# Bardli/RMem_ocu

Measured on AMD Instinct MI355X. Metric: frames/sec (whole node) 480p VOS, N=8 memory bank, higher is better.
Workload: dtype bf16; 1 GPU; davis17_480p_r50_N8; clip_frames=80, job_clips=64, clip_feeder=static, objects=3, memory_bank=1+7, gap=5, clips_in_flight_per_gpu=24, clips_per_group=8, step_unit=batch, parallelism=clip-parallel x1, weights=synthetic (no checkpoint offline), hipgraphs=True, frames_from=HBM, encoder_lookahead=2

## Files before the change

include/rmem.h:

```cpp
#ifndef RMEM_H_
#define RMEM_H_

#include <stddef.h>

#ifdef __cplusplus
extern "C" {
#endif

#define RMEM_ABI_VERSION 15

int rmem_abi_version(void);
const char* rmem_last_error_string(void);

typedef struct rmem_conv_desc {
  int H, W, Cin;
  int Ho, Wo, Cout;
  int KH, KW, stride, pad;
  int ldo;
  int ldr;
  int ld2;
  int relu;
  int out_f32;
  int res_f32;
  int ldx;
// ... 122 lines not shown
  const void* att_long; const void* att_short; float* x;
  const void* w_long; const float* b_long; const void* w_short; const float* b_short; void* tgt3;
  const float* ln3_g; const float* ln3_b; const void* w1; const float* b1; void* h1; float* gn_partial;
} rmem_chain_b_desc;
int rmem_lstt_chain_b(const rmem_chain_b_desc* d, void* stream);
int rmem_lstt_chain_b_merged(const rmem_chain_b_desc* d, const rmem_attn_merge* merge, void* stream);

typedef struct rmem_chain_c_desc {
  int L, clips; float eps; int ld_dec;
  float* x;
  const void* h3; const void* w2; const float* b2; const float* dec_g; const float* dec_b; void* dec_out;
  const float* ln1_g; const float* ln1_b; const void* w_qkv; const float* b_qkv; const float* pos_qk; void* qkv;
} rmem_chain_c_desc;
int rmem_lstt_chain_c(const rmem_chain_c_desc* d, void* stream);

int rmem_layernorm(const void* a, int a_is_f32, int lda, const float* gamma, const float* beta, float eps, int M, int C,
                   void* y_bf16, int ldy, float* y_f32, int ldyf, void* stream);

int rmem_patch_merge_ln(const float* x, int H, int W, int C, const float* gamma, const float* beta, float eps,
                        void* y_bf16, void* stream);
int rmem_patch_merge_ln_images(const float* x, int images, int H, int W, int C, const float* gamma, const float* beta, float eps,
                               void* y_bf16, void* stream);

int rmem_window_attn(const void* qkv, const float* qkv_bias, const float* bias_mask_table, void* out, int H, int W,
                     int C, int heads, int shift, void* stream);
int rmem_window_attn_images(const void* qkv, const float* qkv_bias, const float* bias_mask_table, void* out, int images, int H, int W,
                            int C, int heads, int shift, void* stream);

int rmem_add16(const void* a, const void* b, void* y, long long n, void* stream);
int rmem_add16_grouped(int n, const void* const* a, const void* const* b, void* const* y, long long count, void* stream);
// ... 374 lines not shown
int rmem_mem_read_attn_clips_f16(const void* q, int ldq, const void* k_bank, const void* v_bank, long long slot_stride, int ldkv, const rmem_attn_chunk* chunks, int nchunks, int lk_single, const float* pe_cur, const float* pe_mem, int Lq, int heads, void* out, int ldo, float* attn_mass, int T, int nclips, long long q_clip_stride, long long kv_clip_stride, long long out_clip_stride, void* workspace, void* stream);
int rmem_lstt_attn_pair_clips_f16(const void* q, int ldq, const void* k_bank, const void* v_bank, long long slot_stride, int ldkv, const rmem_attn_chunk* chunks, int nchunks, int lk_total, const float* pe_cur, const float* pe_mem, int Lq, int heads, void* out_long, int ldo, float* attn_mass, int T, int nclips, long long q_clip_stride, long long out_clip_stride, const void* k_short, const void* v_short, int lk_short, long long kv_short_clip_stride, void* out_short, long long out_short_clip_stride, void* workspace, void* stream);
int rmem_lstt_attn_pair_clips_deferred_f16(const void* q, int ldq, const void* k_bank, const void* v_bank, long long slot_stride, int ldkv, const rmem_attn_chunk* chunks, int nchunks, int lk_total, const float* pe_cur, const float* pe_mem, int Lq, int heads, void* out_long, int ldo, float* attn_mass, int T, int nclips, long long q_clip_stride, long long out_clip_stride, const void* k_short, const void* v_short, int lk_short, long long kv_short_clip_stride, void* out_short, long long out_short_clip_stride, void* workspace, rmem_attn_merge* merge, void* stream);
int rmem_layernorm256_f16(const void* a, int a_is_f32, int lda, const void* b, int b_is_f32, int ldb, const float* gamma, const float* beta, float eps, int M, void* y_bf16, int ldy, const float* pos, void* ypos_bf16, int ldyp, float* y_f32, int ldyf, void* stream);
int rmem_layernorm_f16(const void* a, int a_is_f32, int lda, const float* gamma, const float* beta, float eps, int M, int C, void* y_bf16, int ldy, float* y_f32, int ldyf, void* stream);
int rmem_patch_merge_ln_f16(const float* x, int H, int W, int C, const float* gamma, const float* beta, float eps, void* y_bf16, void* stream);
int rmem_window_attn_f16(const void* qkv, const float* qkv_bias, const float* bias_mask_table, void* out, int H, int W, int C, int heads, int shift, void* stream);
int rmem_window_attn_images_f16(const void* qkv, const float* qkv_bias, const float* bias_mask_table, void* out, int images, int H, int W, int C, int heads, int shift, void* stream);
int rmem_patch_merge_ln_images_f16(const float* x, int images, int H, int W, int C, const float* gamma, const float* beta, float eps, void* y_bf16, void* stream);
int rmem_add16_f16(const void* a, const void* b, void* y, long long n, void* stream);
int rmem_add16_grouped_f16(int n, const void* const* a, const void* const* b, void* const* y, long long count, void* stream);
int rmem_lstt_chain_a_f16(const rmem_chain_a_desc* d, void* stream);
int rmem_lstt_chain_b_f16(const rmem_chain_b_desc* d, void* stream);
int rmem_lstt_chain_b_merged_f16(const rmem_chain_b_desc* d, const rmem_attn_merge* merge, void* stream);
int rmem_lstt_chain_c_f16(const rmem_chain_c_desc* d, void* stream);
int rmem_layernorm256_pair_f16(const void* a0, const void* b0, void* y0, const void* a1, const void* b1, void* y1, const float* gamma, const float* beta, float eps, int M, void* stream);
int rmem_bneck_block64_f16(const rmem_bneck_block_desc* desc, const void* x, const void* w1, const float* bias1, const void* w2, const float* bias2, const void* w3, const float* bias3, void* y, const void* w1n, const float* bias1n, void* a_next, void* stream);
int rmem_bneck_chain_f16(const rmem_bneck_chain_desc* desc, const void* b, const void* x2, const void* w3, const float* bias3, const void* res, void* y, const void* w1, const float* bias1, void* a2, void* stream);
int rmem_conv1x1_dual_nhwc_f16(const rmem_conv_desc* desc, const void* x, const void* x2, int H2, int W2, int Cin2, int stride2, const void* w_cat, const float* bias, void* y, void* stream);
int rmem_linear_grouped_f16(const rmem_conv_desc* desc, int n, const void* const* x, const void* const* w, const float* const* bias, const void* const* residual, void* const* y, void* stream);
int rmem_groupnorm_nhwc_f16(const void* x, int M, int C, int groups, const float* gamma, const float* beta, float eps, int act, void* y, float* workspace, void* stream);
int rmem_groupnorm_f32_nhwc_f16(const float* x, int M, int C, int groups, const float* gamma, const float* beta, float eps, int act, void* y, float* workspace, void* stream);
int rmem_groupnorm_nhwc_images_f16(const void* x, int images, int M, int C, int groups, const float* gamma, const float* beta, float eps, int act, void* y, float* workspace, void* stream);
int rmem_groupnorm_head_nhwc_images_f16(const void* x, int images, int M, int C, int groups, const float* gamma, const float* beta, float eps, int act, const void* w, const float* bias, int N, float* y, int ldy, float* workspace, void* stream);
int rmem_gn_act_dwconv5x5_nhwc_images_f16(const void* x, int images, int H, int W, int C, int groups, const float* gamma, const float* beta, float eps, int act, const float* w_t, void* y, float* workspace, void* stream);
int rmem_gn_act_dwconv5x5_prestats_nhwc_images_f16(const void* x, int images, int H, int W, int C, int groups, const float* gamma, const float* beta, float eps, int act, const float* w_t, void* y, const float* stats, void* stream);
int rmem_gn_act_dwconv5x5_nhwc_f16(const void* x, int H, int W, int C, int groups, const float* gamma, const float* beta, float eps, int act, const float* w_t, void* y, float* workspace, void* stream);
int rmem_dwconv5x5_nhwc_f16(const void* x, const float* w_t, void* y, int H, int W, int C, void* stream);
int rmem_image_ptrs_to_nhwc4p_f16(const float* const* img_ptrs, void* out_padded, int images, int H, int W, void* stream);
int rmem_conv3x3_direct_f16(const void* x, int images, int H, int W, int C, const void* w, const float* bias, int relu, void* y, void* stream);
// ... 24 lines not shown
```

rmem_ocu_amd/_lib.py:

```python
from __future__ import annotations

import ctypes as C
import os
import subprocess

_HERE = os.path.dirname(os.path.abspath(__file__))
LIB_PATH = os.environ.get('RMEM_LIB_PATH') or os.path.join(_HERE, 'librmem_hip.so')
ABI_VERSION = 15


class RmemError(RuntimeError):
    pass


class ConvDesc(C.Structure):
    _fields_ = [(n, C.c_int) for n in ('H', 'W', 'Cin', 'Ho', 'Wo', 'Cout', 'KH', 'KW', 'stride', 'pad',
                                       'ldo', 'ldr', 'ld2', 'relu', 'out_f32', 'res_f32', 'ldx', 'batch', 'act_begin',
                                       'res_up_h', 'res_up_w', 'res_up_align')]


class GemmPlan(C.Structure):
    _fields_ = [(n, C.c_int) for n in ('family', 'tile', 'ring', 'is1x1', 'fast', 'splits', 'steps_per_split', 'xcd_ny',
                                       'grid_x', 'grid_y', 'grid_z', 'threads')]

# ... 83 lines not shown
    _fields_ = [('ngroups', _i), ('heads', _i), ('Lq', _i), ('reserved', _i), ('opart', _vp), ('mlg', _vp), ('opart_cs', _ll), ('mlg_cs', _ll)]


def _desc(name, ints, ptrs):
    return type(name, (C.Structure,), {'_fields_': [(ints[0], _i), (ints[1], _i), ('eps', _f), (ints[2], _i)] + [(n, _vp) for n in ptrs]})


ChainA = _desc('ChainA', ('L', 'clips', 'reserved'),
               ('att', 'x', 'w_proj', 'b_proj', 'ln2_g', 'ln2_b', 'curr_v', 'w_q', 'b_q', 'curr_q', 'short_k', 'short_v', 'ln4_g', 'ln4_b',
                'k4', 'v4'))
ChainB = _desc('ChainB', ('L', 'clips', 'gn_splits'),
               ('att_long', 'att_short', 'x', 'w_long', 'b_long', 'w_short', 'b_short', 'tgt3', 'ln3_g', 'ln3_b', 'w1', 'b1', 'h1',
                'gn_partial'))
ChainC = _desc('ChainC', ('L', 'clips', 'ld_dec'),
               ('x', 'h3', 'w2', 'b2', 'dec_g', 'dec_b', 'dec_out', 'ln1_g', 'ln1_b', 'w_qkv', 'b_qkv', 'pos_qk', 'qkv'))
SIGNATURES = {
    'rmem_abi_version': (_i, []),
    'rmem_last_error_string': (C.c_char_p, []),
    'rmem_conv_workspace_bytes': (C.c_size_t, [C.POINTER(ConvDesc)]),
    'rmem_conv2d_nhwc': (_i, [C.POINTER(ConvDesc), _vp, _vp, _vp, _vp, _vp, _vp, _vp, _vp]),
    'rmem_conv_plan': (_i, [C.POINTER(ConvDesc), _i, _i, _i, C.POINTER(GemmPlan)]),
    'rmem_attn_workspace_bytes': (C.c_size_t, [_i, _i, _i]),
    'rmem_mem_read_attn': (_i, [_vp, _i, _vp, _vp, _ll, _i, _vp, _i, _i, _vp, _vp, _i, _i, _vp, _i, _vp, _i, _vp, _vp]),
    'rmem_profile_start': (_i, [_i]),
    'rmem_profile_stop': (_i, [C.POINTER(C.c_double), C.POINTER(C.c_double), C.POINTER(_i)]),
    'rmem_layernorm256': (_i, [_vp, _i, _i, _vp, _i, _i, _vp, _vp, _f, _i, _vp, _i, _vp, _vp, _i, _vp, _i, _vp]),
    'rmem_layernorm': (_i, [_vp, _i, _i, _vp, _vp, _f, _i, _i, _vp, _i, _vp, _i, _vp]),
    'rmem_patch_merge_ln': (_i, [_vp, _i, _i, _i, _vp, _vp, _f, _vp, _vp]),
    'rmem_window_attn': (_i, [_vp, _vp, _vp, _vp, _i, _i, _i, _i, _i, _vp]),
    'rmem_window_attn_images': (_i, [_vp, _vp, _vp, _vp, _i, _i, _i, _i, _i, _i, _vp]),
    'rmem_patch_merge_ln_images': (_i, [_vp, _i, _i, _i, _i, _vp, _vp, _f, _vp, _vp]),
    'rmem_add16': (_i, [_vp, _vp, _vp, _ll, _vp]),
    'rmem_add16_grouped': (_i, [_i, C.POINTER(_vp), C.POINTER(_vp), C.POINTER(_vp), _ll, _vp]),
    'rmem_layernorm256_pair': (_i, [_vp, _vp, _vp, _vp, _vp, _vp, _vp, _vp, _f, _i, _vp]),
    'rmem_lstt_chain_waves': (_i, []),
    'rmem_lstt_chain_rows': (_i, [_i, _i, _i]),
    'rmem_lstt_chain_a': (_i, [C.POINTER(ChainA), _vp]),
    'rmem_lstt_chain_b': (_i, [C.POINTER(ChainB), _vp]),
    'rmem_lstt_chain_b_merged': (_i, [C.POINTER(ChainB), C.POINTER(AttnMerge), _vp]),
    'rmem_lstt_chain_c': (_i, [C.POINTER(ChainC), _vp]),
    'rmem_conv1x1_dual_nhwc': (_i, [C.POINTER(ConvDesc), _vp, _vp, _i, _i, _i, _i, _vp, _vp, _vp, _vp]),
    'rmem_bneck_chain': (_i, [C.POINTER(BneckChainDesc), _vp, _vp, _vp, _vp, _vp, _vp, _vp, _vp, _vp, _vp]),
    'rmem_bneck_block64': (_i, [C.POINTER(BneckBlockDesc), _vp, _vp, _vp, _vp, _vp, _vp, _vp, _vp, _vp, _vp, _vp, _vp]),
    'rmem_linear_grouped': (_i, [C.POINTER(ConvDesc), _i, C.POINTER(_vp), C.POINTER(_vp), C.POINTER(_vp), C.POINTER(_vp), C.POINTER(_vp), _vp]),
    'rmem_groupnorm_workspace_bytes': (C.c_size_t, [_i]),
    'rmem_groupnorm_nhwc': (_i, [_vp, _i, _i, _i, _vp, _vp, _f, _i, _vp, _vp, _vp]),
    'rmem_groupnorm_f32_nhwc': (_i, [_vp, _i, _i, _i, _vp, _vp, _f, _i, _vp, _vp, _vp]),
    'rmem_groupnorm_nhwc_images': (_i, [_vp, _i, _i, _i, _i, _vp, _vp, _f, _i, _vp, _vp, _vp]),
    'rmem_groupnorm_head_nhwc_images': (_i, [_vp, _i, _i, _i, _i, _vp, _vp, _f, _i, _vp, _vp, _i, _vp, _i, _vp, _vp]),
    'rmem_gn_act_dwconv5x5_nhwc_images': (_i, [_vp, _i, _i, _i, _i, _i, _vp, _vp, _f, _i, _vp, _vp, _vp, _vp]),
    'rmem_gn_act_dwconv5x5_prestats_nhwc_images': (_i, [_vp, _i, _i, _i, _i, _i, _vp, _vp, _f, _i, _vp, _vp, _vp, _vp]),
    'rmem_bilinear_nhwc_images': (_i, [_vp, _vp, _i, _i, _i, _i, _i, _i, _i, _vp]),
    'rmem_mem_read_attn_clips': (_i, [_vp, _i, _vp, _vp, _ll, _i, _vp, _i, _i, _vp, _vp, _i, _i, _vp, _i, _vp, _i, _i, _ll, _ll, _ll, _vp, _vp]),
    'rmem_lstt_attn_pair_clips': (_i, [_vp, _i, _vp, _vp, _ll, _i, _vp, _i, _i, _vp, _vp, _i, _i, _vp, _i, _vp, _i, _i, _ll, _ll,
                                       _vp, _vp, _i, _ll, _vp, _ll, _vp, _vp]),
# ... 107 lines not shown
    'rmem_jpeg_entropy_decode': (_i, [_vp, _vp, _i, _i, C.POINTER(JpegPlan), _vp, _vp, _vp, _vp]),
    'rmem_jpeg_coef_to_rgb': (_i, [_vp, _i, _i, C.POINTER(JpegPlan), _vp, _vp, _vp]),
    'rmem_jpeg_decode_batch': (_i, [_vp, _vp, _i, _i, C.POINTER(JpegPlan), _vp, _vp, _vp, _vp, _vp]),
    'rmem_jpeg_encode_header': (_i, [_i, _i, _i, _i, _vp, _i, C.POINTER(_i), _vp]),
    'rmem_jpeg_encode_bound': (C.c_size_t, [_i, _i]),
    'rmem_jpeg_encode_workspace_bytes': (C.c_size_t, [_i, _i, _i]),
    'rmem_jpeg_encode_rgb8': (_i, [_vp, _vp, _vp, _i, _i, _i, _i, _vp, _vp, _vp, _vp, _vp]),
    'rmem_overlay_rgb8': (_i, [_vp, _vp, _vp, _i, _i, _i, _i, _vp, _vp]),
    'rmem_graph_begin': (_i, [_vp]),
    'rmem_graph_end': (_i, [_vp, C.POINTER(_vp)]),
    'rmem_graph_launch': (_i, [_vp, _vp]),
    'rmem_graph_destroy': (_i, [_vp]),
}

F16_TWINS = ('rmem_conv2d_nhwc', 'rmem_mem_read_attn', 'rmem_mem_read_attn_clips', 'rmem_lstt_attn_pair_clips', 'rmem_lstt_attn_pair_clips_deferred', 'rmem_layernorm256', 'rmem_layernorm', 'rmem_patch_merge_ln',
             'rmem_window_attn', 'rmem_window_attn_images', 'rmem_patch_merge_ln_images', 'rmem_add16', 'rmem_add16_grouped', 'rmem_layernorm256_pair', 'rmem_lstt_chain_a', 'rmem_lstt_chain_b', 'rmem_lstt_chain_b_merged', 'rmem_lstt_chain_c', 'rmem_conv1x1_dual_nhwc', 'rmem_bneck_chain', 'rmem_bneck_block64', 'rmem_label_id_embed', 'rmem_image_ptrs_to_nhwc4p', 'rmem_stem7x7s2', 'rmem_stem7x7s2_pool', 'rmem_conv3x3_c64_direct', 'rmem_conv3x3_direct', 'rmem_linear_grouped',
             'rmem_groupnorm_nhwc', 'rmem_groupnorm_f32_nhwc', 'rmem_groupnorm_nhwc_images', 'rmem_groupnorm_head_nhwc_images',
             'rmem_gn_act_dwconv5x5_nhwc_images', 'rmem_gn_act_dwconv5x5_prestats_nhwc_images', 'rmem_gn_act_dwconv5x5_nhwc', 'rmem_dwconv5x5_nhwc', 'rmem_image_to_nhwc8',
             'rmem_image_to_nhwc8_images', 'rmem_image_ptrs_to_nhwc8', 'rmem_ingest_rgb8', 'rmem_maxpool3x3s2_nhwc', 'rmem_maxpool3x3s2_nhwc_images', 'rmem_bilinear_nhwc',
             'rmem_bilinear_nhwc_images', 'rmem_label_to_onehot16', 'rmem_label_to_onehot16_images', 'rmem_gated_attn', 'rmem_local_gated_attn', 'rmem_gated_attn_clips', 'rmem_local_gated_attn_clips')
SIGNATURES.update({n + '_f16': SIGNATURES[n] for n in F16_TWINS})

_lib = None


def build(force: bool = False) -> str:
    src = os.path.join(_HERE, 'csrc')
    if force:
        subprocess.run(['make', '-C', src, 'clean'], check=True, capture_output=True)
    r = subprocess.run(['make', '-C', src, '-j8'], capture_output=True, text=True)
    if r.returncode != 0:
# ... 26 lines not shown
```

rmem_ocu_amd/csrc/rowchain.hip:

```cpp
#include "common.h"
#include "lds_dma.h"
#include "../../include/rmem.h"
#include <stdlib.h>

namespace {

#ifndef RMEM_CHAIN_WAVES
#define RMEM_CHAIN_WAVES 8
#endif
constexpr int NW = RMEM_CHAIN_WAVES;
constexpr int NT = 64 * NW;
constexpr int JT = 16 / NW;
constexpr int WC = 256 / NW;
constexpr int RW = 32 / NW;
constexpr int XS = 260;
constexpr int PF = 16 / JT;

__device__ __forceinline__ f32x4 ld4(const float* p) { return *reinterpret_cast<const f32x4*>(p); }
__device__ __forceinline__ e16x4 cvt4(f32x4 v) { return e16x4{(e16)v[0], (e16)v[1], (e16)v[2], (e16)v[3]}; }
__device__ __forceinline__ f32x4 up4(e16x4 v) { return f32x4{(float)v[0], (float)v[1], (float)v[2], (float)v[3]}; }

typedef __attribute__((ext_vector_type(2))) unsigned u32x2;
typedef __attribute__((ext_vector_type(4))) unsigned u32x4;
#if defined(__HIP_DEVICE_COMPILE__)
__device__ __forceinline__ void st8(rsrc_t r, int off, e16x4 v) { __builtin_amdgcn_raw_buffer_store_b64(__builtin_bit_cast(u32x2, v), r, off, 0, 0); }
__device__ __forceinline__ void st16(rsrc_t r, int off, f32x4 v) { __builtin_amdgcn_raw_buffer_store_b128(__builtin_bit_cast(u32x4, v), r, off, 0, 0); }
#else
__device__ inline void st8(rsrc_t, int, e16x4) {}
__device__ inline void st16(rsrc_t, int, f32x4) {}
#endif

template <int BM, int NP>
__device__ __forceinline__ void stage_tile(e16* A16, int p0, const e16* src, long ld, int nrows) {
  constexpr int NI = NP * BM * 8 / NT;
  static_assert(NP * BM * 8 % NT == 0, "the chunks must divide among the threads");
  const int ch = threadIdx.x & 7;
  e16x8 v[NI];
#pragma unroll
  for (int k = 0; k < NI; ++k) {
    const int i = (threadIdx.x + k * NT) >> 3, row = i % BM;
    v[k] = *reinterpret_cast<const e16x8*>(src + min(row, nrows - 1) * ld + ch * 8 + (i / BM) * 64);
  }
#pragma unroll
  for (int k = 0; k < NI; ++k) {
    const int i = (threadIdx.x + k * NT) >> 3, row = i % BM;
    *reinterpret_cast<e16x8*>(&A16[(p0 + i / BM) * (BM * 64) + swz(row, ch)]) = v[k];
  }
}

template <int BM>
__device__ __forceinline__ void put_a(e16* A16, int p0, int row, int lane, e16x4 v) {
  *reinterpret_cast<e16x4*>(&A16[(p0 + (lane >> 4)) * (BM * 64) + swz(row, (lane & 15) >> 1) + (lane & 1) * 4]) = v;
}

constexpr float MERGE_NEG_BIG = -1.0e30f;
template <int BM>
__device__ __forceinline__ void stage_merged(e16* A16, const rmem_attn_merge& mg, int nrows, int L) {
#pragma clang fp contract(off)
  constexpr int TQ = NT / BM;
  constexpr int HP = TQ >= 8 ? 1 : 8 / TQ;
  constexpr int GP = TQ > 8 ? 64 / TQ : 8;
  const int ql = threadIdx.x % BM, hh = threadIdx.x / BM;
// ... 432 lines not shown
    dump_acc(X, acc, wave, lane);
    if (nb < 2) { wq = wstream((const e16*)d.w_qkv, nb + 1, wave, 8); b_preload(ring, wq, lane); }
    __syncthreads();
#pragma unroll
    for (int h = 0; h < NH; ++h)
#pragma unroll
      for (int rr = 0; rr < RW; ++rr) {
        f32x4 v = ld4(&X[wrow(h, wave, rr) * XS + c0]);
        v += bq[nb];
        v += pos[h].r[rr];
        st8(rqkv, row_off(blk, h, wave, rr, 768, nb * 256 + c0, 2), cvt4(v));
      }
  }
}

#ifndef RMEM_F16
}
extern "C" int rmem_lstt_chain_waves(void) { return NW; }
extern "C" int rmem_lstt_chain_rows(int L, int clips, int cus) { return (long)((L + 31) / 32) * clips > cus ? 64 : 32; }
namespace {
#endif
bool al16(const void* p) { return p == nullptr || ((uintptr_t)p % 16) == 0; }

int chain_rows(int L, int clips) {
  if (const char* e = getenv("RMEM_CHAIN_ROWS")) {
    const int x = atoi(e);
    return x == 32 || x == 64 ? x : 0;
  }
  static int cus = 0;
  if (cus <= 0) {
    int dev = 0, n = 0;
    if (hipGetDevice(&dev) != hipSuccess || hipDeviceGetAttribute(&n, hipDeviceAttributeMultiprocessorCount, dev) != hipSuccess || n <= 0)
      return 32;
    cus = n;
  }
  return rmem_lstt_chain_rows(L, clips, cus);
}

}

extern "C" int RMEM_API(rmem_lstt_chain_a)(const rmem_chain_a_desc* d, void* stream) {
  RMEM_REQUIRE(d && d->L > 0 && d->clips >= 1 && (long)d->L * d->clips < (1L << 20), "rmem_lstt_chain_a: bad geometry (rows must stay below 2^20)");
  RMEM_REQUIRE(d->att && d->x && d->w_proj && d->b_proj && d->ln2_g && d->ln2_b && d->curr_v && d->w_q && d->b_q && d->curr_q && d->short_k &&
               d->short_v && d->ln4_g && d->ln4_b && d->k4 && d->v4, "rmem_lstt_chain_a: null argument");
  RMEM_REQUIRE(al16(d->att) && al16(d->x) && al16(d->w_proj) && al16(d->w_q) && al16(d->curr_v) && al16(d->curr_q) && al16(d->short_k) &&
               al16(d->short_v) && al16(d->k4) && al16(d->v4) && al16(d->b_proj) && al16(d->b_q) && al16(d->ln2_g) && al16(d->ln2_b) &&
               al16(d->ln4_g) && al16(d->ln4_b), "rmem_lstt_chain_a: operands must be 16-byte aligned");
  const int bm = chain_rows(d->L, d->clips);
  RMEM_REQUIRE(bm, "rmem_lstt_chain_a: RMEM_CHAIN_ROWS must be 32 or 64");
  const dim3 grid((d->L + bm - 1) / bm, d->clips);
  if (bm == 64) hipLaunchKernelGGL(k_chain_a<64>, grid, dim3(NT), 0, (hipStream_t)stream, *d);
// ... 53 lines not shown
  const int bm = chain_rows(d->L, d->clips);
  RMEM_REQUIRE(bm, "rmem_lstt_chain_c: RMEM_CHAIN_ROWS must be 32 or 64");
  const dim3 grid((d->L + bm - 1) / bm, d->clips);
  hipStream_t s = (hipStream_t)stream;
  if (bm == 64) {
    if (ffn2 && next) hipLaunchKernelGGL((k_chain_c<64, true, true>), grid, dim3(NT), 0, s, *d);
    else if (ffn2) hipLaunchKernelGGL((k_chain_c<64, true, false>), grid, dim3(NT), 0, s, *d);
    else hipLaunchKernelGGL((k_chain_c<64, false, true>), grid, dim3(NT), 0, s, *d);
  } else {
    if (ffn2 && next) hipLaunchKernelGGL((k_chain_c<32, true, true>), grid, dim3(NT), 0, s, *d);
    else if (ffn2) hipLaunchKernelGGL((k_chain_c<32, true, false>), grid, dim3(NT), 0, s, *d);
    else hipLaunchKernelGGL((k_chain_c<32, false, true>), grid, dim3(NT), 0, s, *d);
  }
  return rmem_check_launch("rmem_lstt_chain_c");
}
```

rmem_ocu_amd/group_runtime.py:

```python
from __future__ import annotations

from typing import Dict, List, Optional, Tuple

import os

import torch

from . import ops
from .encoder_batch import BatchEncoder, SwinBatchEncoder
from .pack import R50_BLOCKS, R50_STRIDES
from .runtime import BF16, D_MODEL, F32, FFN, HEADS, MAX_CHUNKS, PLAIN_CHUNKS, _out, sine_pos_emb, temporal_slots


class GroupRuntime:
    deaot = False
    max_rows = MAX_CHUNKS
    bank_kw = bank_vw = D_MODEL
    dec_cin = 4 * D_MODEL

    def __init__(self, P: Dict[str, torch.Tensor], in_hw: Tuple[int, int], bank_slots: int, device, clips: int,
                 num_lstt: int = 3, align_corners: bool = True, num_classes: int = 11, lookahead: int = 4):
        if ('g0.qvu.w' in P) != self.deaot:
            raise ops.RmemError('GroupRuntime covers the AOTL paths (ResNet-50 / Swin-B), group_runtime_deaot.GroupRuntimeDeAOT the R50-DeAOTL path')
        self.swin = 'pe.w' in P
        self.chain = not os.environ.get('RMEM_NO_CHAIN')
        self.pair_attn = not os.environ.get('RMEM_NO_PAIR_ATTN')
        self.merge_fold = not os.environ.get('RMEM_NO_MERGE_FOLD')
        self.P, self.dev, self.NL, self.B = P, device, num_lstt, clips
        self.dt = P['proj.w'].dtype
        self.align, self.nc = align_corners, num_classes
        H, W = in_hw
        self.H, self.W = H, W
        B = clips
        if self.swin:
            if H % 4 or W % 4:
                raise ops.RmemError('Swin-B path: network size must be a multiple of 4 (the evaluator makes it a multiple of 16)')
            self.H4, self.W4 = H // 4, W // 4
            self.H8, self.W8 = (self.H4 + 1) // 2, (self.W4 + 1) // 2
            self.H16, self.W16 = (self.H8 + 1) // 2, (self.W8 + 1) // 2
            self.enc_ch = (128, 256, 512)
        else:
            self.H2, self.W2 = _out(H, 7, 2, 3), _out(W, 7, 2, 3)
# ... 326 lines not shown
            o = [ops.label_id_embed(labels, P['idbank.w'], P['idbank.b'], self.lab_net, self.id_emb, Hs=hs, Ws=ws, H=self.H, W=self.W, K=k,
                                    stride=s, pad=p, ncls=self.nc, images=B)]
        else:
            o = [ops.label_to_onehot16(labels, self.onehot, Hs=hs, Ws=ws, Hd=self.H, Wd=self.W, ncls=self.nc, images=B)]
            o.append(self._conv(self.onehot, P['idbank.w'], P['idbank.b'], self.id_emb, H=self.H, W=self.W, Cin=16, Cout=D_MODEL,
                                KH=k, KW=k, stride=s, pad=p))
        self._prog[key] = o
        return o

    def prog_update(self, append: bool) -> list:
        key = f'update_{int(append)}'
        if key in self._prog:
            return self._prog[key]
        P, NL, L, C, B = self.P, self.NL, self.L, D_MODEL, self.B
        R = B * L
        o = [ops.add16_grouped(self.tgt3 + (self.curr_V if append else []), [self.id_emb] * (NL * (2 if append else 1)),
                                  self.tmpA + (self.tmpB if append else []), R * C)]
        w = lambda nm: [P[f'l{i}.{nm}.w'] for i in range(NL)]
        b = lambda nm: [P[f'l{i}.{nm}.b'] for i in range(NL)]
        o.append(ops.linear_grouped(self.tgt3, w('linear_QMem'), b('linear_QMem'), self.short_K, M=R, K=C, N=C))
        o.append(ops.linear_grouped(self.tmpA, w('linear_VMem'), b('linear_VMem'), self.short_V, M=R, K=C, N=C))
        if append:
            o.append(ops.linear_grouped(self.tmpB, w('linear_V'), b('linear_V'), self.new_V, M=R, K=C, N=C))
            for i in range(NL):
                o.append(self._scatter(self.curr_Q[i], self.bank_K[i]))
                o.append(self._scatter(self.new_V[i], self.bank_V[i]))
        self._prog[key] = o
        return o


# ... 6 lines not shown
```

rmem_ocu_amd/ops.py:

```python
from __future__ import annotations

import ctypes as C
import os
from typing import Dict, Optional, Sequence

import torch

from . import _lib
from ._lib import AttnChunk, ConvDesc, RmemError

BF16 = torch.bfloat16
F16 = torch.float16
F32 = torch.float32
E16 = (BF16, F16)


def _fn(name: str, dt):
    if dt not in E16:
        raise RmemError(f'{name}: 16-bit operands must be bfloat16 or float16, got {dt}')
    return getattr(_lib.lib(), name + ('_f16' if dt == F16 else ''))


def _first16(*ts):
    for t in ts:
# ... 199 lines not shown
                  dict(att_long=att_long, att_short=att_short, x=x, w_long=w_long, b_long=b_long, w_short=w_short, b_short=b_short, tgt3=tgt3,
                       ln3_g=ln3[0], ln3_b=ln3[1], w1=w1, b1=b1, h1=h1, gn_partial=gn_partial), dt, () if merge is None else (merge,))


def lstt_chain_c(*, L, clips, x, dt, h3=None, w2=None, b2=None, dec_norm=(None, None), dec_out=None, ld_dec=0, ln1=(None, None), w_qkv=None,
                 b_qkv=None, pos_qk=None, qkv=None, eps=1e-5) -> Op:
    R = clips * L
    assert x.dtype == F32 and x.numel() >= R * 256
    assert h3 is None or (h3.dtype == dt and h3.numel() >= R * 1024 and w2.numel() == 262144 and dec_out.numel() >= (R - 1) * ld_dec + 256)
    assert w_qkv is None or (w_qkv.numel() == 196608 and pos_qk.dtype == F32 and pos_qk.numel() >= R * 768 and qkv.dtype == dt and qkv.numel() >= R * 768)
    return _chain('rmem_lstt_chain_c', _lib.ChainC, (L, clips, eps, ld_dec),
                  dict(x=x, h3=h3, w2=w2, b2=b2, dec_g=dec_norm[0], dec_b=dec_norm[1], dec_out=dec_out, ln1_g=ln1[0], ln1_b=ln1[1], w_qkv=w_qkv,
                       b_qkv=b_qkv, pos_qk=pos_qk, qkv=qkv), dt)


def attn_workspace(Lq: int, heads: int, nchunks: int, device, nclips: int = 1) -> torch.Tensor:
    n = nclips * _lib.lib().rmem_attn_workspace_bytes(Lq, heads, nchunks)
    return torch.empty(n // 4, dtype=F32, device=device)


def make_chunk_table(chunks: Sequence[Sequence[int]]) -> torch.Tensor:
    t = torch.zeros(len(chunks), 8, dtype=torch.int32)
    for i, c in enumerate(chunks):
        t[i, :5] = torch.tensor(list(c), dtype=torch.int32)
    return t


def mem_read_attn(q, k_bank, v_bank, out, workspace, *, Lq, heads=8, ldq, ldkv, ldo, slot_stride=0, chunks=None,
                  nchunks=1, lk_single=0, pe_cur=None, pe_mem=None, mass=None, T=0, nclips=1, q_cs=0, kv_cs=0, out_cs=0) -> Op:
    _dev(q, k_bank, v_bank, out, workspace, chunks, pe_cur, pe_mem, mass)
# ... 493 lines not shown
```

rmem_ocu_amd/pack.py:

```python
from __future__ import annotations

from typing import Dict

import torch

import threading

BN_EPS = 1e-5
_DT = torch.bfloat16
_PACK_LOCK = threading.Lock()
R50_BLOCKS = (3, 4, 6)
R50_STRIDES = (1, 2, 2)


def _conv_w(w: torch.Tensor, cin_pad: int = 0) -> torch.Tensor:
    cout, cin, kh, kw = w.shape
    w = w.permute(0, 2, 3, 1)
    if cin_pad and cin_pad > cin:
        w = torch.nn.functional.pad(w, (0, cin_pad - cin))
    return w.contiguous().to(_DT)


def pack_frag(w: torch.Tensor, waves: int = 0) -> torch.Tensor:
    if not waves:
# ... 136 lines not shown
        norm(d + '.ln1', s + '.norm1')
        put(d + '.self_qk.w', torch.cat([sd[s + '.self_attn.linear_Q.weight'], sd[s + '.self_attn.linear_K.weight']], 0).float().to(_DT))
        put(d + '.self_qk.b', torch.cat([sd[s + '.self_attn.linear_Q.bias'], sd[s + '.self_attn.linear_K.bias']], 0).float())
        put(d + '.self_qkv.w', torch.cat([sd[s + '.self_attn.linear_Q.weight'], sd[s + '.self_attn.linear_K.weight'],
                                          sd[s + '.self_attn.linear_V.weight']], 0).float().to(_DT))
        put(d + '.self_qkv.b', torch.cat([sd[s + '.self_attn.linear_Q.bias'], sd[s + '.self_attn.linear_K.bias'],
                                          sd[s + '.self_attn.linear_V.bias']], 0).float())
        lin(d + '.self_proj', s + '.self_attn.projection')
        norm(d + '.ln2', s + '.norm2')
        for nm in ('linear_Q', 'linear_V', 'linear_QMem', 'linear_VMem', 'linear1', 'linear2'):
            lin(f'{d}.{nm}', f'{s}.{nm}')
        norm(d + '.ln4', s + '.norm4')
        lin(d + '.long_proj', s + '.long_term_attn.projection')
        lin(d + '.short_proj', s + '.short_term_attn.projection')
        norm(d + '.ln3', s + '.norm3')
        for nm in ('self_proj', 'linear_Q', 'long_proj', 'short_proj', 'linear1', 'linear2', 'self_qkv'):
            put(f'{d}.{nm}.wf', pack_frag(P[f'{d}.{nm}.w']))
        norm(d + '.gn', s + '.activation.gn')
        put(d + '.dw.w', sd[s + '.activation.conv.weight'].float().view(-1, 25).t())
        norm(f'dec_norm{i}', f'LSTT.decoder_norms.{i}')

    for nm in ('conv_in', 'conv_16x', 'conv_8x', 'conv_4x'):
        put(f'dec.{nm}.w', _conv_w(sd[f'decoder.{nm}.conv.weight'].float())); put(f'dec.{nm}.b', sd[f'decoder.{nm}.conv.bias'].float())
        norm(f'dec.{nm}.gn', f'decoder.{nm}.gn')
    for nm in ('adapter_16x', 'adapter_8x', 'adapter_4x', 'conv_out'):
        put(f'dec.{nm}.w', _conv_w(sd[f'decoder.{nm}.weight'].float())); put(f'dec.{nm}.b', sd[f'decoder.{nm}.bias'].float())

    put('idbank.w', _conv_w(sd['patch_wise_id_bank.weight'].float(), cin_pad=16)); put('idbank.b', sd['patch_wise_id_bank.bias'].float())
    put('pe_cur', sd['cur_pos_emb'].float().view(-1)); put('pe_mem', sd['mem_pos_emb'].float())
    return P
```

Before: 3480 frames/s.

## Fuse LSTT memory-update linears, id add and bank append into one chain kernel

```diff
diff --git a/include/rmem.h b/include/rmem.h
--- a/include/rmem.h
+++ b/include/rmem.h
@@ -160,6 +160,15 @@
 } rmem_chain_c_desc;
 int rmem_lstt_chain_c(const rmem_chain_c_desc* d, void* stream);
 
+typedef struct rmem_chain_u_desc {
+  int L, clips, layers, append;
+  long long slot_stride; const int* append_slots; const void* id_emb;
+  const void* tgt3[4]; const void* curr_v[4]; const void* curr_q[4];
+  void* short_k[4]; void* short_v[4]; void* new_v[4]; void* bank_k[4]; void* bank_v[4];
+  const void* w_qmem[4]; const float* b_qmem[4]; const void* w_vmem[4]; const float* b_vmem[4]; const void* w_v[4]; const float* b_v[4];
+} rmem_chain_u_desc;
+int rmem_lstt_chain_update(const rmem_chain_u_desc* d, void* stream);
+
 int rmem_layernorm(const void* a, int a_is_f32, int lda, const float* gamma, const float* beta, float eps, int M, int C,
                    void* y_bf16, int ldy, float* y_f32, int ldyf, void* stream);
 
@@ -564,6 +573,7 @@
 int rmem_lstt_chain_b_f16(const rmem_chain_b_desc* d, void* stream);
 int rmem_lstt_chain_b_merged_f16(const rmem_chain_b_desc* d, const rmem_attn_merge* merge, void* stream);
 int rmem_lstt_chain_c_f16(const rmem_chain_c_desc* d, void* stream);
+int rmem_lstt_chain_update_f16(const rmem_chain_u_desc* d, void* stream);
 int rmem_layernorm256_pair_f16(const void* a0, const void* b0, void* y0, const void* a1, const void* b1, void* y1, const float* gamma, const float* beta, float eps, int M, void* stream);
 int rmem_bneck_block64_f16(const rmem_bneck_block_desc* desc, const void* x, const void* w1, const float* bias1, const void* w2, const float* bias2, const void* w3, const float* bias3, void* y, const void* w1n, const float* bias1n, void* a_next, void* stream);
 int rmem_bneck_chain_f16(const rmem_bneck_chain_desc* desc, const void* b, const void* x2, const void* w3, const float* bias3, const void* res, void* y, const void* w1, const float* bias1, void* a2, void* stream);
diff --git a/rmem_ocu_amd/_lib.py b/rmem_ocu_amd/_lib.py
--- a/rmem_ocu_amd/_lib.py
+++ b/rmem_ocu_amd/_lib.py
@@ -121,6 +121,15 @@
                 'gn_partial'))
 ChainC = _desc('ChainC', ('L', 'clips', 'ld_dec'),
                ('x', 'h3', 'w2', 'b2', 'dec_g', 'dec_b', 'dec_out', 'ln1_g', 'ln1_b', 'w_qkv', 'b_qkv', 'pos_qk', 'qkv'))
+
+
+class ChainU(C.Structure):
+    PER_LAYER = ('tgt3', 'curr_v', 'curr_q', 'short_k', 'short_v', 'new_v', 'bank_k', 'bank_v', 'w_qmem', 'b_qmem', 'w_vmem', 'b_vmem',
+                 'w_v', 'b_v')
+    _fields_ = [('L', _i), ('clips', _i), ('layers', _i), ('append', _i), ('slot_stride', _ll), ('append_slots', _vp), ('id_emb', _vp)] + \
+               [(n, _vp * 4) for n in PER_LAYER]
+
+
 SIGNATURES = {
     'rmem_abi_version': (_i, []),
     'rmem_last_error_string': (C.c_char_p, []),
@@ -146,6 +155,7 @@
     'rmem_lstt_chain_b': (_i, [C.POINTER(ChainB), _vp]),
     'rmem_lstt_chain_b_merged': (_i, [C.POINTER(ChainB), C.POINTER(AttnMerge), _vp]),
     'rmem_lstt_chain_c': (_i, [C.POINTER(ChainC), _vp]),
+    'rmem_lstt_chain_update': (_i, [C.POINTER(ChainU), _vp]),
     'rmem_conv1x1_dual_nhwc': (_i, [C.POINTER(ConvDesc), _vp, _vp, _i, _i, _i, _i, _vp, _vp, _vp, _vp]),
     'rmem_bneck_chain': (_i, [C.POINTER(BneckChainDesc), _vp, _vp, _vp, _vp, _vp, _vp, _vp, _vp, _vp, _vp]),
     'rmem_bneck_block64': (_i, [C.POINTER(BneckBlockDesc), _vp, _vp, _vp, _vp, _vp, _vp, _vp, _vp, _vp, _vp, _vp, _vp]),
@@ -283,7 +293,7 @@
 }
 
 F16_TWINS = ('rmem_conv2d_nhwc', 'rmem_mem_read_attn', 'rmem_mem_read_attn_clips', 'rmem_lstt_attn_pair_clips', 'rmem_lstt_attn_pair_clips_deferred', 'rmem_layernorm256', 'rmem_layernorm', 'rmem_patch_merge_ln',
-             'rmem_window_attn', 'rmem_window_attn_images', 'rmem_patch_merge_ln_images', 'rmem_add16', 'rmem_add16_grouped', 'rmem_layernorm256_pair', 'rmem_lstt_chain_a', 'rmem_lstt_chain_b', 'rmem_lstt_chain_b_merged', 'rmem_lstt_chain_c', 'rmem_conv1x1_dual_nhwc', 'rmem_bneck_chain', 'rmem_bneck_block64', 'rmem_label_id_embed', 'rmem_image_ptrs_to_nhwc4p', 'rmem_stem7x7s2', 'rmem_stem7x7s2_pool', 'rmem_conv3x3_c64_direct', 'rmem_conv3x3_direct', 'rmem_linear_grouped',
+             'rmem_window_attn', 'rmem_window_attn_images', 'rmem_patch_merge_ln_images', 'rmem_add16', 'rmem_add16_grouped', 'rmem_layernorm256_pair', 'rmem_lstt_chain_a', 'rmem_lstt_chain_b', 'rmem_lstt_chain_b_merged', 'rmem_lstt_chain_c', 'rmem_lstt_chain_update', 'rmem_conv1x1_dual_nhwc', 'rmem_bneck_chain', 'rmem_bneck_block64', 'rmem_label_id_embed', 'rmem_image_ptrs_to_nhwc4p', 'rmem_stem7x7s2', 'rmem_stem7x7s2_pool', 'rmem_conv3x3_c64_direct', 'rmem_conv3x3_direct', 'rmem_linear_grouped',
              'rmem_groupnorm_nhwc', 'rmem_groupnorm_f32_nhwc', 'rmem_groupnorm_nhwc_images', 'rmem_groupnorm_head_nhwc_images',
              'rmem_gn_act_dwconv5x5_nhwc_images', 'rmem_gn_act_dwconv5x5_prestats_nhwc_images', 'rmem_gn_act_dwconv5x5_nhwc', 'rmem_dwconv5x5_nhwc', 'rmem_image_to_nhwc8',
              'rmem_image_to_nhwc8_images', 'rmem_image_ptrs_to_nhwc8', 'rmem_ingest_rgb8', 'rmem_maxpool3x3s2_nhwc', 'rmem_maxpool3x3s2_nhwc_images', 'rmem_bilinear_nhwc',
diff --git a/rmem_ocu_amd/csrc/rowchain.hip b/rmem_ocu_amd/csrc/rowchain.hip
--- a/rmem_ocu_amd/csrc/rowchain.hip
+++ b/rmem_ocu_amd/csrc/rowchain.hip
@@ -31,21 +31,34 @@
 #endif
 
 template <int BM, int NP>
+struct Tile {
+  static_assert(NP * BM * 8 % NT == 0, "the chunks must divide among the threads");
+  static constexpr int NI = NP * BM * 8 / NT;
+  e16x8 v[NI];
+};
+template <int BM, int NP>
+__device__ __forceinline__ Tile<BM, NP> load_tile(const e16* src, long ld, int nrows) {
+  const int ch = threadIdx.x & 7;
+  Tile<BM, NP> t;
+#pragma unroll
+  for (int k = 0; k < Tile<BM, NP>::NI; ++k) {
+    const int i = (threadIdx.x + k * NT) >> 3, row = i % BM;
+    t.v[k] = *reinterpret_cast<const e16x8*>(src + min(row, nrows - 1) * ld + ch * 8 + (i / BM) * 64);
+  }
+  return t;
+}
+template <int BM, int NP>
+__device__ __forceinline__ void put_tile(e16* A16, int p0, const Tile<BM, NP>& t) {
+  const int ch = threadIdx.x & 7;
+#pragma unroll
+  for (int k = 0; k < Tile<BM, NP>::NI; ++k) {
+    const int i = (threadIdx.x + k * NT) >> 3, row = i % BM;
+    *reinterpret_cast<e16x8*>(&A16[(p0 + i / BM) * (BM * 64) + swz(row, ch)]) = t.v[k];
+  }
+}
+template <int BM, int NP>
 __device__ __forceinline__ void stage_tile(e16* A16, int p0, const e16* src, long ld, int nrows) {
-  constexpr int NI = NP * BM * 8 / NT;
-  static_assert(NP * BM * 8 % NT == 0, "the chunks must divide among the threads");
-  const int ch = threadIdx.x & 7;
-  e16x8 v[NI];
-#pragma unroll
-  for (int k = 0; k < NI; ++k) {
-    const int i = (threadIdx.x + k * NT) >> 3, row = i % BM;
-    v[k] = *reinterpret_cast<const e16x8*>(src + min(row, nrows - 1) * ld + ch * 8 + (i / BM) * 64);
-  }
-#pragma unroll
-  for (int k = 0; k < NI; ++k) {
-    const int i = (threadIdx.x + k * NT) >> 3, row = i % BM;
-    *reinterpret_cast<e16x8*>(&A16[(p0 + i / BM) * (BM * 64) + swz(row, ch)]) = v[k];
-  }
+  put_tile<BM, NP>(A16, p0, load_tile<BM, NP>(src, ld, nrows));
 }
 
 template <int BM>
@@ -508,6 +521,127 @@
   }
 }
 
+constexpr int OS = 260;
+
+template <int NI>
+__device__ __forceinline__ void add_id(e16x8 (&o)[NI], const e16x8 (&a)[NI], const e16x8 (&b)[NI]) {
+#pragma unroll
+  for (int k = 0; k < NI; ++k)
+#pragma unroll
+    for (int j = 0; j < 8; ++j) o[k][j] = (e16)((float)a[k][j] + (float)b[k][j]);
+}
+
+template <int MT>
+__device__ __forceinline__ void put_out(e16* O, const f32x4 (&acc)[MT][JT], const float (&bias)[JT], int wave, int lane) {
+  const int fr = lane & 15, fc = lane >> 4;
+#pragma unroll
+  for (int i = 0; i < MT; ++i)
+#pragma unroll
+    for (int j = 0; j < JT; ++j)
+#pragma unroll
+      for (int q = 0; q < 4; ++q) O[(i * 16 + fc * 4 + q) * OS + wave * WC + j * 16 + fr] = (e16)(acc[i][j][q] + bias[j]);
+}
+
+template <int BM>
+__device__ __forceinline__ void store_out(const e16* O, rsrc_t r, const Blk& blk, int wave, int lane) {
+#pragma unroll
+  for (int h = 0; h < BM / 32; ++h)
+#pragma unroll
+    for (int rr = 0; rr < RW; ++rr)
+      st8(r, row_off(blk, h, wave, rr, 256, lane * 4, 2), *reinterpret_cast<const e16x4*>(&O[wrow(h, wave, rr) * OS + lane * 4]));
+}
+
+__device__ __forceinline__ void load_bias(float (&b)[JT], const float* bias, int wave, int lane) {
+#pragma unroll
+  for (int j = 0; j < JT; ++j) b[j] = bias[wave * WC + j * 16 + (lane & 15)];
+}
+
+template <int BM, bool APPEND>
+__global__ __launch_bounds__(NT) void k_chain_u(rmem_chain_u_desc d) {
+  constexpr int MT = BM / 16, PANEL = BM * 64;
+  typedef Tile<BM, 4> T4;
+  __shared__ __attribute__((aligned(16))) char smem[4 * PANEL * 2 + BM * OS * 2];
+  e16* A16 = reinterpret_cast<e16*>(smem);
+  e16* O = reinterpret_cast<e16*>(smem + 4 * PANEL * 2);
+  const int lane = threadIdx.x & 63, wave = __builtin_amdgcn_readfirstlane(threadIdx.x >> 6);
+  const Blk blk = my_rows<BM>(d.L);
+  const Blk inclip = {blk.nrows, (long)blockIdx.x * BM};
+  const long rows = (long)d.clips * d.L;
+  const int l0 = gridDim.z > 1 ? blockIdx.z : 0, l1 = gridDim.z > 1 ? l0 + 1 : d.layers;
+  const int slot = APPEND ? d.append_slots[blockIdx.y] : -1;
+  const long slot_off = slot >= 0 ? slot * d.slot_stride : 0, slot_bytes = slot >= 0 ? (long)d.L * 512 : 0;
+  const T4 id = load_tile<BM, 4>((const e16*)d.id_emb + blk.g0 * 256, 256, blk.nrows);
+  T4 t = load_tile<BM, 4>((const e16*)d.tgt3[l0] + blk.g0 * 256, 256, blk.nrows);
+  BRing ring;
+  f32x4 acc[MT][JT];
+  const e16* w = wstream((const e16*)d.w_qmem[l0], 0, wave, 8);
+  b_preload(ring, w, lane);
+  for (int l = l0; l < l1; ++l) {
+    const rsrc_t rsk = make_rsrc(d.short_k[l], rows * 512), rsv = make_rsrc(d.short_v[l], rows * 512);
+    float bqm[JT], bvm[JT], bv[JT];
+    load_bias(bqm, d.b_qmem[l], wave, lane);
+    load_bias(bvm, d.b_vmem[l], wave, lane);
+    T4 cv, cq;
+    if (APPEND) {
+      load_bias(bv, d.b_v[l], wave, lane);
+      cv = load_tile<BM, 4>((const e16*)d.curr_v[l] + blk.g0 * 256, 256, blk.nrows);
+      cq = load_tile<BM, 4>((const e16*)d.curr_q[l] + blk.g0 * 256, 256, blk.nrows);
+    }
+    put_tile<BM, 4>(A16, 0, t);
+    __syncthreads();
+    zero_acc(acc);
+    gemm_rows<BM, 4>(A16, 0, w, ring, acc, lane);
+    w = wstream((const e16*)d.w_vmem[l], 0, wave, 8);
+    b_preload(ring, w, lane);
+    __syncthreads();
+    {
+      T4 s;
+      add_id(s.v, t.v, id.v);
+      put_tile<BM, 4>(A16, 0, s);
+    }
+    put_out(O, acc, bqm, wave, lane);
+    if (l + 1 < l1) t = load_tile<BM, 4>((const e16*)d.tgt3[l + 1] + blk.g0 * 256, 256, blk.nrows);
+    __syncthreads();
+    store_out<BM>(O, rsk, blk, wave, lane);
+    zero_acc(acc);
+    gemm_rows<BM, 4>(A16, 0, w, ring, acc, lane);
+    if (APPEND || l + 1 < l1) {
+      w = wstream((const e16*)(APPEND ? d.w_v[l] : d.w_qmem[l + 1]), 0, wave, 8);
+      b_preload(ring, w, lane);
+    }
+    __syncthreads();
+    put_out(O, acc, bvm, wave, lane);
+    if (APPEND) {
+      T4 s;
+      add_id(s.v, cv.v, id.v);
+      put_tile<BM, 4>(A16, 0, s);
+    }
+    __syncthreads();
+    store_out<BM>(O, rsv, blk, wave, lane);
+    if (APPEND) {
+      const rsrc_t rnv = make_rsrc(d.new_v[l], rows * 512);
+      const rsrc_t rbk = make_rsrc((const e16*)d.bank_k[l] + slot_off, slot_bytes), rbv = make_rsrc((const e16*)d.bank_v[l] + slot_off, slot_bytes);
+#pragma unroll
+      for (int k = 0; k < T4::NI; ++k) {
+        const int i = (threadIdx.x + k * NT) >> 3, row = i % BM;
+        const int off = row < blk.nrows ? (int)(((inclip.g0 + row) * 256 + (i / BM) * 64 + (threadIdx.x & 7) * 8) * 2) : OOB;
+        st16(rbk, off, __builtin_bit_cast(f32x4, cq.v[k]));
+      }
+      zero_acc(acc);
+      gemm_rows<BM, 4>(A16, 0, w, ring, acc, lane);
+      if (l + 1 < l1) {
+        w = wstream((const e16*)d.w_qmem[l + 1], 0, wave, 8);
+        b_preload(ring, w, lane);
+      }
+      __syncthreads();
+      put_out(O, acc, bv, wave, lane);
+      __syncthreads();
+      store_out<BM>(O, rnv, blk, wave, lane);
+      store_out<BM>(O, rbv, inclip, wave, lane);
+    }
+  }
+}
+
 #ifndef RMEM_F16
 }
 extern "C" int rmem_lstt_chain_waves(void) { return NW; }
@@ -516,19 +650,24 @@
 #endif
 bool al16(const void* p) { return p == nullptr || ((uintptr_t)p % 16) == 0; }
 
+int device_cus() {
+  static int cus = 0;
+  if (cus <= 0) {
+    int dev = 0, n = 0;
+    if (hipGetDevice(&dev) != hipSuccess || hipDeviceGetAttribute(&n, hipDeviceAttributeMultiprocessorCount, dev) != hipSuccess || n <= 0)
+      return 0;
+    cus = n;
+  }
+  return cus;
+}
+
 int chain_rows(int L, int clips) {
   if (const char* e = getenv("RMEM_CHAIN_ROWS")) {
     const int x = atoi(e);
     return x == 32 || x == 64 ? x : 0;
   }
-  static int cus = 0;
-  if (cus <= 0) {
-    int dev = 0, n = 0;
-    if (hipGetDevice(&dev) != hipSuccess || hipDeviceGetAttribute(&n, hipDeviceAttributeMultiprocessorCount, dev) != hipSuccess || n <= 0)
-      return 32;
-    cus = n;
-  }
-  return rmem_lstt_chain_rows(L, clips, cus);
+  const int cus = device_cus();
+  return cus ? rmem_lstt_chain_rows(L, clips, cus) : 32;
 }
 
 }
@@ -612,3 +751,36 @@
   }
   return rmem_check_launch("rmem_lstt_chain_c");
 }
+
+extern "C" int RMEM_API(rmem_lstt_chain_update)(const rmem_chain_u_desc* d, void* stream) {
+  RMEM_REQUIRE(d && d->L > 0 && d->clips >= 1 && (long)d->L * d->clips < (1L << 20), "rmem_lstt_chain_update: bad geometry (rows must stay below 2^20)");
+  RMEM_REQUIRE(d->layers >= 1 && d->layers <= 4, "rmem_lstt_chain_update: 1 to 4 layers");
+  RMEM_REQUIRE(d->id_emb && al16(d->id_emb), "rmem_lstt_chain_update: id_emb must be given and 16-byte aligned");
+  const bool append = d->append != 0;
+  RMEM_REQUIRE(!append || (d->append_slots && d->slot_stride >= (long long)d->L * 256 && d->slot_stride % 8 == 0),
+               "rmem_lstt_chain_update: an append needs append_slots and slot_stride >= L * 256 elements (a multiple of 8)");
+  for (int i = 0; i < d->layers; ++i) {
+    RMEM_REQUIRE(d->tgt3[i] && d->short_k[i] && d->short_v[i] && d->w_qmem[i] && d->b_qmem[i] && d->w_vmem[i] && d->b_vmem[i],
+                 "rmem_lstt_chain_update: null argument");
+    RMEM_REQUIRE(al16(d->tgt3[i]) && al16(d->short_k[i]) && al16(d->short_v[i]) && al16(d->w_qmem[i]) && al16(d->w_vmem[i]),
+                 "rmem_lstt_chain_update: operands must be 16-byte aligned");
+    if (!append) continue;
+    RMEM_REQUIRE(d->curr_v[i] && d->curr_q[i] && d->new_v[i] && d->bank_k[i] && d->bank_v[i] && d->w_v[i] && d->b_v[i],
+                 "rmem_lstt_chain_update: null argument of an append");
+    RMEM_REQUIRE(al16(d->curr_v[i]) && al16(d->curr_q[i]) && al16(d->new_v[i]) && al16(d->bank_k[i]) && al16(d->bank_v[i]) && al16(d->w_v[i]),
+                 "rmem_lstt_chain_update: operands must be 16-byte aligned");
+  }
+  const int bm = chain_rows(d->L, d->clips);
+  RMEM_REQUIRE(bm, "rmem_lstt_chain_update: RMEM_CHAIN_ROWS must be 32 or 64");
+  const int nx = (d->L + bm - 1) / bm;
+  const dim3 grid(nx, d->clips, (long)nx * d->clips * d->layers <= device_cus() ? d->layers : 1);
+  hipStream_t s = (hipStream_t)stream;
+  if (bm == 64) {
+    if (append) hipLaunchKernelGGL((k_chain_u<64, true>), grid, dim3(NT), 0, s, *d);
+    else hipLaunchKernelGGL((k_chain_u<64, false>), grid, dim3(NT), 0, s, *d);
+  } else {
+    if (append) hipLaunchKernelGGL((k_chain_u<32, true>), grid, dim3(NT), 0, s, *d);
+    else hipLaunchKernelGGL((k_chain_u<32, false>), grid, dim3(NT), 0, s, *d);
+  }
+  return rmem_check_launch("rmem_lstt_chain_update");
+}
diff --git a/rmem_ocu_amd/group_runtime.py b/rmem_ocu_amd/group_runtime.py
--- a/rmem_ocu_amd/group_runtime.py
+++ b/rmem_ocu_amd/group_runtime.py
@@ -26,6 +26,7 @@
         self.chain = not os.environ.get('RMEM_NO_CHAIN')
         self.pair_attn = not os.environ.get('RMEM_NO_PAIR_ATTN')
         self.merge_fold = not os.environ.get('RMEM_NO_MERGE_FOLD')
+        self.update_chain = os.environ.get('RMEM_NO_UPDATE_CHAIN') != '1'
         self.P, self.dev, self.NL, self.B = P, device, num_lstt, clips
         self.dt = P['proj.w'].dtype
         self.align, self.nc = align_corners, num_classes
@@ -382,6 +383,14 @@
             return self._prog[key]
         P, NL, L, C, B = self.P, self.NL, self.L, D_MODEL, self.B
         R = B * L
+        if self.chain and self.update_chain:
+            p = lambda nm, k: [P[f'l{i}.{nm}.{k}'] for i in range(NL)]
+            kw = dict(curr_v=self.curr_V, curr_q=self.curr_Q, new_v=self.new_V, bank_k=self.bank_K, bank_v=self.bank_V,
+                      w_v=p('linear_V', 'wf'), b_v=p('linear_V', 'b'), append_slots=self.append_slots, slot_stride=L * C) if append else {}
+            self._prog[key] = [ops.lstt_chain_update(L=L, clips=B, id_emb=self.id_emb, tgt3=self.tgt3, short_k=self.short_K, short_v=self.short_V,
+                                                     w_qmem=p('linear_QMem', 'wf'), b_qmem=p('linear_QMem', 'b'),
+                                                     w_vmem=p('linear_VMem', 'wf'), b_vmem=p('linear_VMem', 'b'), **kw)]
+            return self._prog[key]
         o = [ops.add16_grouped(self.tgt3 + (self.curr_V if append else []), [self.id_emb] * (NL * (2 if append else 1)),
                                   self.tmpA + (self.tmpB if append else []), R * C)]
         w = lambda nm: [P[f'l{i}.{nm}.w'] for i in range(NL)]
diff --git a/rmem_ocu_amd/ops.py b/rmem_ocu_amd/ops.py
--- a/rmem_ocu_amd/ops.py
+++ b/rmem_ocu_amd/ops.py
@@ -237,6 +237,34 @@
                        b_qkv=b_qkv, pos_qk=pos_qk, qkv=qkv), dt)
 
 
+def lstt_chain_update(*, L, clips, id_emb, tgt3, short_k, short_v, w_qmem, b_qmem, w_vmem, b_vmem, curr_v=None, curr_q=None, new_v=None,
+                      bank_k=None, bank_v=None, w_v=None, b_v=None, append_slots=None, slot_stride=0) -> Op:
+    dt = id_emb.dtype
+    R, n = clips * L, len(tgt3)
+    append = curr_v is not None
+    per_layer = dict(tgt3=tgt3, curr_v=curr_v, curr_q=curr_q, short_k=short_k, short_v=short_v, new_v=new_v, bank_k=bank_k, bank_v=bank_v,
+                     w_qmem=w_qmem, b_qmem=b_qmem, w_vmem=w_vmem, b_vmem=b_vmem, w_v=w_v, b_v=b_v)
+    only_append = ('curr_v', 'curr_q', 'new_v', 'bank_k', 'bank_v', 'w_v', 'b_v')
+    assert 1 <= n <= 4 and all((v is not None and len(v) == n) if (append or k not in only_append) else v is None for k, v in per_layer.items())
+    rows = [id_emb, *tgt3, *short_k, *short_v] + ([*curr_v, *curr_q, *new_v] if append else [])
+    assert all(t.dtype == dt and t.numel() >= R * 256 for t in rows)
+    ws = [*w_qmem, *w_vmem] + (list(w_v) if append else [])
+    bs = [*b_qmem, *b_vmem] + (list(b_v) if append else [])
+    assert all(t.dtype == dt and t.numel() == 65536 for t in ws) and all(t.dtype == F32 and t.numel() == 256 for t in bs)
+    if append:
+        assert append_slots is not None and append_slots.dtype == torch.int32 and append_slots.numel() >= clips
+        assert slot_stride >= L * 256 and all(t.dtype == dt and t.numel() >= slot_stride for t in (*bank_k, *bank_v))
+    ts = [id_emb, append_slots] + [t for v in per_layer.values() if v is not None for t in v]
+    _dev(*ts)
+    for t in ts:
+        if t is not None and t.data_ptr() % 16:
+            raise RmemError('rmem_lstt_chain_update: operands must be 16-byte aligned')
+    arr = lambda v: (C.c_void_p * 4)(*[_ptr(t) for t in v]) if v is not None else (C.c_void_p * 4)()
+    d = _lib.ChainU(int(L), int(clips), n, int(append), int(slot_stride), _ptr(append_slots), _ptr(id_emb),
+                    *[arr(per_layer[k]) for k in _lib.ChainU.PER_LAYER])
+    return Op(_fn('rmem_lstt_chain_update', dt), (C.byref(d),), 'rmem_lstt_chain_update', (d, ts))
+
+
 def attn_workspace(Lq: int, heads: int, nchunks: int, device, nclips: int = 1) -> torch.Tensor:
     n = nclips * _lib.lib().rmem_attn_workspace_bytes(Lq, heads, nchunks)
     return torch.empty(n // 4, dtype=F32, device=device)
diff --git a/rmem_ocu_amd/pack.py b/rmem_ocu_amd/pack.py
--- a/rmem_ocu_amd/pack.py
+++ b/rmem_ocu_amd/pack.py
@@ -174,7 +174,7 @@
         lin(d + '.long_proj', s + '.long_term_attn.projection')
         lin(d + '.short_proj', s + '.short_term_attn.projection')
         norm(d + '.ln3', s + '.norm3')
-        for nm in ('self_proj', 'linear_Q', 'long_proj', 'short_proj', 'linear1', 'linear2', 'self_qkv'):
+        for nm in ('self_proj', 'linear_Q', 'long_proj', 'short_proj', 'linear1', 'linear2', 'self_qkv', 'linear_QMem', 'linear_VMem', 'linear_V'):
             put(f'{d}.{nm}.wf', pack_frag(P[f'{d}.{nm}.w']))
         norm(d + '.gn', s + '.activation.gn')
         put(d + '.dw.w', sd[s + '.activation.conv.weight'].float().view(-1, 25).t())
```

Measured after the change: 3503 frames/s, median of 6. No clear change (+0.7%).
